# Shinokawa/Fast-SCNN-pytorch

Hardware: AMD Instinct MI355X
Metric: images/sec fwd+bwd @1024x2048 bs=8 per GPU; 1/2/4/8-GPU scaling (higher is better)
Workload: dtype bf16; 1 GPU; cfg3 train step: fwd + CE(ignore -1) + bwd + fused SGD (fused low-res upsample+CE head); model=FastSCNN (19 classes), global_batch=8, per_gpu_batch=8, parallelism=dp1

## Files before the change

### fast-scnn-pytorch_amd/_lib.py

```python
import ctypes
import os
import threading

_HERE = os.path.dirname(os.path.abspath(__file__))
LIB_PATH = os.environ.get("FSCNN_LIB", os.path.join(_HERE, "libfastscnn_hip.so"))

DT_F32, DT_BF16, DT_F16 = 0, 1, 2
DT_U8 = 3

c_int, c_ll, c_float, c_vp, c_char_p = (ctypes.c_int, ctypes.c_longlong, ctypes.c_float,
                                        ctypes.c_void_p, ctypes.c_char_p)
c_ull, c_double = ctypes.c_ulonglong, ctypes.c_double
P_int, P_ll, P_vp = ctypes.POINTER(c_int), ctypes.POINTER(c_ll), ctypes.POINTER(c_vp)
P_float = ctypes.POINTER(c_float)
P_double = ctypes.POINTER(c_double)
c_uint, P_ubyte = ctypes.c_uint, ctypes.POINTER(ctypes.c_ubyte)


class AuxHead(ctypes.Structure):
    _fields_ = [("head", c_int), ("aux_weight", c_float), ("ignore_index", c_ll),
                ("smooth", c_float), ("dice_weight", c_float), ("focal_weight", c_float),
                ("alpha", c_float), ("gamma", c_float), ("thresh", c_float), ("min_kept", c_ll),
                ("class_weight", c_vp)]

# ... 146 lines not shown
                                       c_vp]),
    "fscnn_block_ir_fwd": (c_int, [c_vp, c_int, c_int, c_int, c_int, c_int, c_int, c_int, c_int,
                                   c_vp, c_vp, c_vp, c_vp, c_vp, c_vp, c_vp, c_vp, c_vp, c_int,
                                   c_vp, c_int, c_vp]),
    "fscnn_pyramid_pool_bwd": (c_int, [c_vp, c_int, c_int, c_int, c_int, c_int, c_vp, c_int,
                                       c_int, c_vp]),
    "fscnn_bn_apply": (c_int, [c_ll, c_int, c_vp, c_int, c_vp, c_vp, c_vp, c_int, c_vp, c_vp, c_vp,
                               c_int, c_int, c_vp, c_int, c_int, c_vp]),
    "fscnn_bn_bwd": (c_int, [c_ll, c_int, c_vp, c_int, c_vp, c_int, c_vp, c_vp, c_vp, c_vp, c_vp,
                             c_int, c_int, c_vp, c_vp, c_vp, c_vp, c_vp, c_vp, c_vp, c_vp, c_vp,
                             c_vp, c_vp, c_vp, c_vp, c_int, P_int, P_int, c_vp]),
    "fscnn_ppm_branches_ok": (c_int, [c_int, c_int, c_int]),
    "fscnn_ppm_branches_fwd": (c_int, [c_int, P_int, c_int, c_vp, c_vp, c_vp, c_vp, c_vp, c_vp,
                                       c_vp, c_float, c_vp, c_vp, c_int, c_vp, c_vp, c_vp, c_vp,
                                       c_int, c_vp]),
    "fscnn_ppm_branches_bwd": (c_int, [c_int, P_int, c_int, c_vp, c_int, c_vp, c_int, c_vp, c_vp,
                                       c_vp, c_vp, c_vp, c_vp, c_vp, c_vp, c_vp, c_vp, c_vp, c_int,
                                       c_vp]),
    "fscnn_ppm_up_fwd": (c_int, [c_vp, c_int, c_int, c_int, c_int, c_vp, c_int, c_int, c_vp]),
    "fscnn_ppm_up_bwd": (c_int, [c_vp, c_int, c_int, c_int, c_int, c_int, c_int, c_vp, c_vp]),
    "fscnn_dropout": (c_int, [c_vp, c_int, c_int, c_int, c_int, c_int, c_int, c_ull, c_vp, c_ull,
                              c_float, c_vp, c_vp, c_vp, c_int, c_vp]),
    "fscnn_dw3x3_parts": (c_int, [c_int, c_int, c_int, c_int, c_int, c_int, c_int]),
    "fscnn_dw3x3_fwd_train": (c_int, [c_vp, c_int, c_int, c_int, c_int, c_int, c_int, c_vp, c_vp,
                                      c_vp, c_vp, c_vp, c_vp, c_vp, c_vp, c_vp, c_vp, c_vp, c_vp,
                                      c_float, c_vp, c_vp, c_vp, c_vp, P_int, c_vp]),
    "fscnn_dw3x3_dgrad_bn": (c_int, [c_vp, c_int, c_int, c_int, c_int, c_int, c_int, c_vp, c_vp,
                                     c_vp, c_vp, c_vp, c_vp, c_vp, c_int, c_vp, c_vp, c_vp, c_vp,
                                     c_vp, c_vp, P_int, c_vp]),
    "fscnn_dw3x3_wgrad_train": (c_int, [c_vp, c_vp, c_int, c_int, c_int, c_int, c_int, c_int,
                                        c_vp, c_vp, c_vp, c_vp, c_vp]),
    "fscnn_pw_fwd_train_route": (c_int, [c_int, c_int, c_int, c_int, c_int, c_int, c_int, P_int]),
    "fscnn_pw_fwd_train": (c_int, [c_int, c_int, c_int, c_vp, c_int, c_vp, c_vp, c_vp, c_int, c_vp,
                                   c_vp, c_int, c_vp, c_vp, c_vp, c_vp, c_vp, c_vp, c_vp, c_vp,
                                   c_float, c_vp, c_vp, c_vp, c_vp, c_int, P_int, P_int, c_vp]),
    "fscnn_pw_wgrad_train": (c_int, [c_int, c_int, c_int, c_vp, c_int, c_vp, c_int, c_vp, c_vp,
                                     c_vp, c_vp, c_vp, c_vp, c_int, P_int, c_vp]),
    "fscnn_pw_dgrad_train_route": (c_int, [c_int, c_int, c_int, c_int, c_int, c_int, c_int, c_int,
                                           P_int]),
    "fscnn_pw_dgrad_train": (c_int, [c_int, c_int, c_int, c_vp, c_int, c_vp, c_int, c_vp, c_int,
                                     c_vp, c_int, c_vp, c_int, c_vp, c_vp, c_vp, c_vp, c_int,
                                     c_vp, c_vp, c_vp, c_vp, c_vp, c_vp, c_vp, c_int, c_float,
                                     c_ull, c_ull, c_vp, c_int, P_int, P_int, c_vp]),
    "fscnn_im2col3": (c_int, [c_vp, c_int, c_int, c_int, c_int, c_int, c_int, c_vp, c_int, c_vp]),
    "fscnn_col2im3": (c_int, [c_vp, c_int, c_int, c_int, c_int, c_int, c_int, c_vp, c_int, c_int,
                              c_vp]),
# ... 74 lines not shown
```

### fast-scnn-pytorch_amd/csrc/capi.cpp

```cpp
#include <algorithm>
#include <chrono>
#include <cmath>
#include <cstdlib>
#include <cstdarg>
#include <cstdio>
#include <cstring>
#include <new>
#include <string>

#include "../../include/fastscnn.h"
#include "net.hpp"

namespace fscnn {

static thread_local char g_err[512] = "";

void set_error(const char* fmt, ...) {
  va_list ap;
  va_start(ap, fmt);
  vsnprintf(g_err, sizeof g_err, fmt, ap);
  va_end(ap);
}
const char* last_error() { return g_err; }

// ... 1541 lines not shown
  d.y = y; d.ldy = ldy; d.seed = seed; d.p = p; d.seed_add = seed_add;
  d.seed_ptr = reinterpret_cast<const uint64_t*>(seed_slot);
  return dropout(d, dtype, S(stream));
}

static int dw_train_check(const char* who, int dtype, int N, int H, int W, int C, int stride) {
  if (!dt_ok(dtype)) {
    set_error("%s: dtype %d", who, dtype);
    return E_INVALID;
  }
  const int V = vec_w(dtype);
  if (N < 1 || H < 1 || W < 1 || C < 1 || C % V || (stride != 1 && stride != 2)) {
    set_error("%s: N=%d H=%d W=%d C=%d stride=%d (C a multiple of %d, stride 1 or 2)", who, N, H,
              W, C, stride, V);
    return E_INVALID;
  }
  return OK;
}

int fscnn_dw3x3_parts(int N, int H, int W, int C, int stride, int dtype, int dgrad) {
  if (dw_train_check("fscnn_dw3x3_parts", dtype, N, H, W, C, stride)) return -1;
  if (dgrad) return dw_dgrad_parts(N, H, W, C, dtype, stride);
  return dw_parts(N, (H - 1) / stride + 1, (W - 1) / stride + 1, C, dtype, stride);
}

int fscnn_dw3x3_fwd_train(const void* x, int dtype, int N, int H, int W, int C, int stride,
                          const float* w, const float* in_scale, const float* in_shift, void* z,
                          float* part, unsigned* counters, double* tsum, const float* gamma,
                          const float* beta, float* rmean, float* rvar, long long* nbt,
                          float momentum, float* mean, float* invstd, float* scale, float* shift,
                          int* in_kernel, void* stream) {
  if (!x || !w || !z || !part || !counters || !tsum || !gamma || !beta || !rmean || !rvar ||
      !mean || !invstd || !scale || !shift || ((in_scale != nullptr) != (in_shift != nullptr))) {
    set_error("fscnn_dw3x3_fwd_train: null argument (in_scale and in_shift come together)");
    return E_INVALID;
  }
  const int rc = dw_train_check("fscnn_dw3x3_fwd_train", dtype, N, H, W, C, stride);
  if (rc) return rc;
  DwArgs d{};
  d.N = N; d.H = H; d.W = W; d.C = C; d.stride = stride;
  d.Ho = (H - 1) / stride + 1; d.Wo = (W - 1) / stride + 1;
  d.x = x; d.w = w; d.in_scale = in_scale; d.in_shift = in_shift;
  d.relu = 0; d.y = z;
  d.part = part;
  d.tail.counters = counters;
  d.tail.tsum = tsum;
// ... 526 lines not shown
```

### fast-scnn-pytorch_amd/csrc/dwconv.hip

```cpp
#include "bn_finish.hpp"

#include <optional>

namespace fscnn {

constexpr int DWL_CB = 8;

template <typename T, int S> struct DwCfg;
template <> struct DwCfg<float, 1> { static constexpr int HS = 2, WS = 4, GX = 8, GY = 4; };
template <> struct DwCfg<float, 2> { static constexpr int HS = 1, WS = 2, GX = 8, GY = 4; };
template <> struct DwCfg<bf16, 1> { static constexpr int HS = 2, WS = 4, GX = 4, GY = 4; };
template <> struct DwCfg<bf16, 2> { static constexpr int HS = 2, WS = 2, GX = 4, GY = 4; };
template <int S> struct DwCfg<f16, S> : DwCfg<bf16, S> {};
template <typename T, int S> struct DwTile {
  static constexpr int HS = DwCfg<T, S>::HS, WS = DwCfg<T, S>::WS;
  static constexpr int GX = DwCfg<T, S>::GX, GY = DwCfg<T, S>::GY, G = GX * GY;
  static constexpr int QPV = VecW<T>::V / 4;
  static constexpr int TH = GY * HS, TW = GX * WS;
  static constexpr int IR = (TH - 1) * S + 3, IC = (TW - 1) * S + 3;
  static constexpr int LPT = (IR * IC + QPV * G - 1) / (QPV * G);
  static constexpr int NR = (HS - 1) * S + 3, NC = (WS - 1) * S + 3;
};

__device__ __forceinline__ void quad_ld(const float* p, float (&v)[4]) {
// ... 56 lines not shown
    const int r = pix / G::IC, col = pix - r * G::IC;
    const int hi = hi0 + r, wi = wi0 + col;
    const bool ok = pix < G::IR * G::IC && hi >= 0 && hi < H && wi >= 0 && wi < W;
    const size_t off = ok ? (((size_t)n * H + hi) * W + wi) * C + (size_t)(cvbase + lv) * V : 0;
    raw[k] = sel4(ok, *reinterpret_cast<const uint4*>(x + off));
  }
#pragma unroll
  for (int k = 0; k < G::LPT; ++k) {
    const int i = tid + k * nthr;
    if (i < G::IR * G::IC * cbv) {
      uint4 v = raw[k];
      if constexpr (IT) {
        const int pix = i / cbv;
        const int r = pix / G::IC, col = pix - r * G::IC;
        const int hi = hi0 + r, wi = wi0 + col;
        const bool ok = hi >= 0 && hi < H && wi >= 0 && wi < W;
        v = sel4(ok, bnrelu_vec<T>(v, sc, sh));
      }
      s_in[i] = v;
    }
  }
}

template <typename T, int S, bool FLIP, bool IT, bool BR = false, bool TL = false>
__global__ __launch_bounds__(256, 3) void dw_fwd_kernel(DwArgs a, int cbv) {
  using G = DwTile<T, S>;
  extern __shared__ __attribute__((aligned(16))) uint4 s_dyn[];
  uint4* s_in = s_dyn;
  float* s_red = reinterpret_cast<float*>(s_dyn + G::IR * G::IC * cbv);
  const int tid = threadIdx.x, nthr = blockDim.x;
  const int QB = cbv * G::QPV;
  const int q = tid % QB, grp = tid / QB;
  const int gx = grp % G::GX, gy = grp / G::GX;
  int bx, by, bz;
  dw_tile(bx, by, bz);
  const int tiles_h = cdiv(a.Ho, G::TH);
  const int n = bz / tiles_h;
  const int th0 = (bz - n * tiles_h) * G::TH, tw0 = by * G::TW;
  const int c0 = bx * cbv * VecW<T>::V + q * 4;
  stamp(a.stamps, 0);
  dw_stage<T, S, IT>(s_in, (const T*)a.x, a.H, a.W, a.C, n, th0 * S - 1, tw0 * S - 1,
                     bx * cbv, cbv, tid, nthr, a.in_scale, a.in_shift);
  float wt[9][4];
#pragma unroll
  for (int j = 0; j < 4; ++j)
#pragma unroll
    for (int t = 0; t < 9; ++t) wt[FLIP ? 8 - t : t][j] = a.w[(size_t)(c0 + j) * 9 + t];
  __syncthreads();
  stamp(a.stamps, 1);

  const T* sl = reinterpret_cast<const T*>(s_in);
  const int pstride = cbv * VecW<T>::V;
  float acc[G::HS][G::WS][4];
#pragma unroll
  for (int r = 0; r < G::HS; ++r)
#pragma unroll
    for (int p = 0; p < G::WS; ++p)
#pragma unroll
      for (int j = 0; j < 4; ++j) acc[r][p][j] = 0.f;
  const int lr0 = gy * G::HS * S, lc0 = gx * G::WS * S;
#pragma unroll
  for (int rr = 0; rr < G::NR; ++rr) {
    asm volatile("" ::: "memory");
#pragma unroll
    for (int ci = 0; ci < G::NC; ++ci) {
      float v[4];
      quad_ld(sl + ((lr0 + rr) * G::IC + lc0 + ci) * pstride + q * 4, v);
#pragma unroll
      for (int r = 0; r < G::HS; ++r) {
        const int kh = rr - r * S;
        if (kh < 0 || kh > 2) continue;
#pragma unroll
        for (int p = 0; p < G::WS; ++p) {
          const int kw = ci - p * S;
          if (kw < 0 || kw > 2) continue;
#pragma unroll
          for (int j = 0; j < 4; ++j) acc[r][p][j] = fmaf(v[j], wt[kh * 3 + kw][j], acc[r][p][j]);
        }
      }
    }
  }

  const int ho0 = th0 + gy * G::HS, wo0 = tw0 + gx * G::WS;
  const int nrow = max(0, min(G::HS, a.Ho - ho0)), ncol = max(0, min(G::WS, a.Wo - wo0));
  {
    float sc[4], sh[4];
#pragma unroll
    for (int j = 0; j < 4; ++j) {
      sc[j] = a.scale ? a.scale[c0 + j] : 1.f;
      sh[j] = a.scale ? a.shift[c0 + j] : 0.f;
    }
#pragma unroll
    for (int r = 0; r < G::HS; ++r) {
      if (r >= nrow) continue;
      T* yb = (T*)a.y + (((size_t)n * a.Ho + ho0 + r) * a.Wo + wo0) * a.C + c0;
#pragma unroll
      for (int p = 0; p < G::WS; ++p) {
        if (p >= ncol) continue;
        float o[4];
#pragma unroll
        for (int j = 0; j < 4; ++j) {
          const float t = acc[r][p][j] * sc[j] + sh[j];
          o[j] = a.relu ? fmaxf(t, 0.f) : t;
          acc[r][p][j] = round_as<T>(o[j]);
        }
        quad_st(yb + (size_t)p * a.C, o);
      }
    }
  }
  stamp(a.stamps, 2);
  if constexpr (BR) {
    const BnBwdPart& b = a.bs;
    const bool m2 = b.mode == 2;
    float bm[4], bi[4], bsc[4], bsh[4], s1[4], s2[4];
#pragma unroll
    for (int j = 0; j < 4; ++j) {
      bm[j] = b.mean[c0 + j];
      bi[j] = b.invstd[c0 + j];
      bsc[j] = m2 ? b.scale[c0 + j] : 0.f;
      bsh[j] = m2 ? b.shift[c0 + j] : 1.f;
      s1[j] = s2[j] = 0.f;
    }
#pragma unroll
    for (int r = 0; r < G::HS; ++r) {
      float z[G::WS][4];
#pragma unroll
      for (int p = 0; p < G::WS; ++p) {
        const bool ok = r < nrow && p < ncol;
        const size_t pix = ok ? ((size_t)n * a.Ho + ho0 + r) * a.Wo + wo0 + p : 0;
        quad_ld((const T*)b.z + pix * a.C + c0, z[p]);
      }
#pragma unroll
      for (int p = 0; p < G::WS; ++p) {
        const bool ok = r < nrow && p < ncol;
#pragma unroll
        for (int j = 0; j < 4; ++j) {
          float gv = round_as<T>(acc[r][p][j]);
          gv = (ok && fmaf(z[p][j], bsc[j], bsh[j]) > 0.f) ? gv : 0.f;
          s1[j] += gv;
          s2[j] += gv * (z[p][j] - bm[j]) * bi[j];
        }
      }
      asm volatile("" ::: "memory");
    }
    float* rec = b.part + ((size_t)bz * gridDim.y + by) * 2 * a.C;
#pragma unroll
    for (int pass = 0; pass < 2; ++pass) {
      __syncthreads();
#pragma unroll
      for (int j = 0; j < 4; ++j) s_red[(grp * QB + q) * 4 + j] = pass ? s2[j] : s1[j];
      __syncthreads();
      if (grp == 0) {
#pragma unroll
        for (int j = 0; j < 4; ++j) {
          float t = 0.f;
          for (int g2 = 0; g2 < G::G; ++g2) t += s_red[(g2 * QB + q) * 4 + j];
          st_wt(rec + (size_t)pass * a.C + c0 + j, t);
        }
      }
    }
    stamp(a.stamps, 3);
    if constexpr (TL)
      tail_finish<false>(b.part, gridDim.y * gridDim.z, a.C, bz * gridDim.y + by,
                         bx * cbv * VecW<T>::V, cbv * VecW<T>::V, bx, a.tail,
                         reinterpret_cast<double*>(s_dyn));
    stamp(a.stamps, 4);
    return;
  }
  if (a.part == nullptr) return;
  const int trows = min(G::TH, a.Ho - th0), tcols = min(G::TW, a.Wo - tw0);
  const float cnt = (float)(trows * tcols);
  float mean[4];
#pragma unroll
  for (int j = 0; j < 4; ++j) {
    float sum = 0.f;
#pragma unroll
    for (int r = 0; r < G::HS; ++r)
#pragma unroll
      for (int p = 0; p < G::WS; ++p) sum += (r < nrow && p < ncol) ? acc[r][p][j] : 0.f;
    s_red[(grp * QB + q) * 4 + j] = sum;
  }
  __syncthreads();
#pragma unroll
  for (int j = 0; j < 4; ++j) {
    float sum = 0.f;
    for (int g = 0; g < G::G; ++g) sum += s_red[(g * QB + q) * 4 + j];
    mean[j] = sum / cnt;
  }
  __syncthreads();
#pragma unroll
  for (int j = 0; j < 4; ++j) {
    float m2 = 0.f;
#pragma unroll
    for (int r = 0; r < G::HS; ++r)
#pragma unroll
      for (int p = 0; p < G::WS; ++p) {
        const float d = acc[r][p][j] - mean[j];
        m2 += (r < nrow && p < ncol) ? d * d : 0.f;
      }
    s_red[(grp * QB + q) * 4 + j] = m2;
  }
  __syncthreads();
  if (grp == 0) {
    float* rec = a.part + ((size_t)bz * gridDim.y + by) * 3 * a.C;
#pragma unroll
    for (int j = 0; j < 4; ++j) {
      float m2 = 0.f;
      for (int g = 0; g < G::G; ++g) m2 += s_red[(g * QB + q) * 4 + j];
      st_wt(rec + c0 + j, mean[j]);
      st_wt(rec + a.C + c0 + j, m2);
      st_wt(rec + 2 * a.C + c0 + j, cnt);
    }
  }
  stamp(a.stamps, 3);
  if constexpr (TL)
    tail_finish<true>(a.part, gridDim.y * gridDim.z, a.C, bz * gridDim.y + by,
                      bx * cbv * VecW<T>::V, cbv * VecW<T>::V, bx, a.tail,
                      reinterpret_cast<double*>(s_dyn));
  stamp(a.stamps, 4);
}

template <typename T, int S>
static size_t dw_shm(int cbv) {
  using G = DwTile<T, S>;
  return (size_t)G::IR * G::IC * cbv * 16 + (size_t)cbv * 32 * 16;
}

static dim3 dw_grid(int N, int Ho, int Wo, int C, int V, int S, int& cbv) {
  cbv = dw_cbv(C / V);
  int TH, TW;
  if (V == 4) {
    TH = S == 1 ? DwTile<float, 1>::TH : DwTile<float, 2>::TH;
    TW = S == 1 ? DwTile<float, 1>::TW : DwTile<float, 2>::TW;
  } else {
    TH = S == 1 ? DwTile<bf16, 1>::TH : DwTile<bf16, 2>::TH;
    TW = S == 1 ? DwTile<bf16, 1>::TW : DwTile<bf16, 2>::TW;
  }
  return dim3(C / V / cbv, cdiv(Wo, TW), N * cdiv(Ho, TH));
}

int dw_parts(int N, int Ho, int Wo, int C, int dtype, int stride) {
  int cbv;
  dim3 g = dw_grid(N, Ho, Wo, C, dtype == DT_F32 ? 4 : 8, stride, cbv);
  return (int)(g.y * g.z);
}

template <typename T, bool FLIP, bool IT, bool BR>
static void dw_launch_fwd_t(const DwArgs& a, dim3 grid, int nthr, int cbv, hipStream_t st) {
  if constexpr (BR) {
    if (a.tail_ink) prof_launch(dw_fwd_kernel<T, 1, true, false, true, true>, grid, nthr, dw_shm<T, 1>(cbv), st, a, cbv);
    else prof_launch(dw_fwd_kernel<T, 1, true, false, true>, grid, nthr, dw_shm<T, 1>(cbv), st, a, cbv);
    return;
  }
  if (!FLIP && a.tail_ink) {
    if (a.stride == 1) prof_launch(dw_fwd_kernel<T, 1, false, IT, false, true>, grid, nthr, dw_shm<T, 1>(cbv), st, a, cbv);
    else prof_launch(dw_fwd_kernel<T, 2, false, IT, false, true>, grid, nthr, dw_shm<T, 2>(cbv), st, a, cbv);
    return;
  }
  if (a.stride == 1) prof_launch(dw_fwd_kernel<T, 1, FLIP, IT>, grid, nthr, dw_shm<T, 1>(cbv), st, a, cbv);
  else prof_launch(dw_fwd_kernel<T, 2, FLIP, IT>, grid, nthr, dw_shm<T, 2>(cbv), st, a, cbv);
}

template <bool FLIP, bool IT, bool BR = false>
static int dw_launch_fwd(const DwArgs& a, int dtype, hipStream_t st) {
  const int V = dtype == DT_F32 ? 4 : 8;
  int cbv;
  dim3 grid = dw_grid(a.N, a.Ho, a.Wo, a.C, V, a.stride, cbv);
  if (grid.z > 65535 || grid.y > 65535) {
    set_error("dw: grid too large (%u x %u)", grid.y, grid.z);
    return E_UNSUPPORTED;
  }
  const int nthr = cbv * 32;
  DwArgs as = a;
  as.stamps = stamp_region();
  if (dtype == DT_F32) dw_launch_fwd_t<float, FLIP, IT, BR>(as, grid, nthr, cbv, st);
  else if (dtype == DT_F16) dw_launch_fwd_t<f16, FLIP, IT, BR>(as, grid, nthr, cbv, st);
  else dw_launch_fwd_t<bf16, FLIP, IT, BR>(as, grid, nthr, cbv, st);
  return check_launch(FLIP ? "dw_dgrad" : "dw_fwd");
}

int dw_fwd_tail_ink(const DwArgs& a, int dtype, int* P) {
  int cbv;
  const dim3 g = dw_grid(a.N, a.Ho, a.Wo, a.C, dtype == DT_F32 ? 4 : 8, a.stride, cbv);
// ... 248 lines not shown
    else DWD2(bf16);
#undef DWD2
    rc = check_launch("dw_dgrad");
  }
  if (rc || !fin || ink) return rc;
  ps.reset();
  return bn_bwd_finalize(a.bs.part, P, a.C, a.tail.count, a.tail.dgamma, a.tail.dbeta,
                         a.tail.coef, st, a.tail.counters, a.tail.tab);
}

int dw_dgrad_parts(int N, int H, int W, int C, int dtype, int stride) {
  const int V = dtype == DT_F32 ? 4 : 8;
  if (stride == 1) {
    int cbv;
    const dim3 g = dw_grid(N, H, W, C, V, 1, cbv);
    return (int)(g.y * g.z);
  }
  int bx, by;
  dw_block_shape(C, DWD2_V, bx, by);
  const int gy = cdiv(W, by * 4), NB = N * ((H + 1) / 2);
  return gy * cdiv(NB, dwd2_rpw(gy, NB));
}

template <typename T, int S, bool IT>
__global__ __launch_bounds__(256, 2) void dw_wgrad_kernel(DwBwdArgs a, int cbv, int tpb) {
  using G = DwTile<T, S>;
  extern __shared__ __attribute__((aligned(16))) uint4 s_in[];
  const int tid = threadIdx.x, nthr = blockDim.x;
  const int QB = cbv * G::QPV;
  const int q = tid % QB, grp = tid / QB;
  const int gx = grp % G::GX, gy = grp / G::GX;
  int bx, by, bz;
  dw_tile(bx, by, bz);
  const int tiles_h = cdiv(a.Ho, G::TH), tiles_w = cdiv(a.Wo, G::TW);
  const int n = bz / tiles_h;
  const int th0 = (bz - n * tiles_h) * G::TH;
  const int c0 = bx * cbv * VecW<T>::V + q * 4;
  const int ho0 = th0 + gy * G::HS;
  const int nrow = max(0, min(G::HS, a.Ho - ho0));
  const T* sl = reinterpret_cast<const T*>(s_in);
  const int pstride = cbv * VecW<T>::V;
  float acc[9][4];
#pragma unroll
  for (int t = 0; t < 9; ++t)
#pragma unroll
    for (int j = 0; j < 4; ++j) acc[t][j] = 0.f;
  const int tw_lo = by * tpb, tw_hi = min(tiles_w, tw_lo + tpb);
  for (int twi = tw_lo; twi < tw_hi; ++twi) {
    const int tw0 = twi * G::TW;
    const int wo0 = tw0 + gx * G::WS;
    const int ncol = max(0, min(G::WS, a.Wo - wo0));
    float g[G::HS][G::WS][4];
    const T* gb = (const T*)a.dy + c0;
#pragma unroll
    for (int r = 0; r < G::HS; ++r)
#pragma unroll
      for (int p = 0; p < G::WS; ++p) {
        const bool ok = r < nrow && p < ncol;
        const size_t off = ok ? (((size_t)n * a.Ho + ho0 + r) * a.Wo + wo0 + p) * a.C : 0;
        quad_ld(gb + off, g[r][p]);
      }
#pragma unroll
    for (int r = 0; r < G::HS; ++r)
#pragma unroll
      for (int p = 0; p < G::WS; ++p) {
        const bool ok = r < nrow && p < ncol;
#pragma unroll
        for (int j = 0; j < 4; ++j) g[r][p][j] = ok ? g[r][p][j] : 0.f;
      }
    __syncthreads();
    dw_stage<T, S, IT>(s_in, (const T*)a.x, a.H, a.W, a.C, n, th0 * S - 1, tw0 * S - 1, bx * cbv,
                       cbv, tid, nthr, a.x_scale, a.x_shift);
    __syncthreads();
    const int lr0 = gy * G::HS * S, lc0 = gx * G::WS * S;
#pragma unroll
    for (int rr = 0; rr < G::NR; ++rr)
#pragma unroll
      for (int ci = 0; ci < G::NC; ++ci) {
        float v[4];
        quad_ld(sl + ((lr0 + rr) * G::IC + lc0 + ci) * pstride + q * 4, v);
#pragma unroll
        for (int r = 0; r < G::HS; ++r) {
          const int kh = rr - r * S;
          if (kh < 0 || kh > 2) continue;
#pragma unroll
          for (int p = 0; p < G::WS; ++p) {
            const int kw = ci - p * S;
            if (kw < 0 || kw > 2) continue;
#pragma unroll
            for (int j = 0; j < 4; ++j)
              acc[kh * 3 + kw][j] = fmaf(v[j], g[r][p][j], acc[kh * 3 + kw][j]);
          }
        }
      }
  }
// ... 23 lines not shown
  long long tpb = blocks / 1024;
  if (tpb < 1) tpb = 1;
  if (tpb > tiles_w) tpb = tiles_w;
  grid.y = (unsigned)cdiv((int)tiles_w, (int)tpb);
  return (int)tpb;
}

int dw_wgrad_parts(int N, int Ho, int Wo, int C, int dtype, int stride) {
  dim3 g;
  int cbv;
  dw_wgrad_tpb(N, Ho, Wo, C, dtype == DT_F32 ? 4 : 8, stride, g, cbv);
  return (int)(g.y * g.z);
}

int dw_wgrad(const DwBwdArgs& a, int dtype, hipStream_t st) {
  const int V = dtype == DT_F32 ? 4 : 8;
  dim3 grid;
  int cbv;
  const int tpb = dw_wgrad_tpb(a.N, a.Ho, a.Wo, a.C, V, a.stride, grid, cbv);
  const double E = dtype == DT_F32 ? 4.0 : 2.0;
  const double in_el = (double)a.N * a.C * a.H * a.W, out_el = (double)a.N * a.C * a.Ho * a.Wo;
  ProfScope ps(PK_DW_WGRAD, st, E * (in_el + out_el), 18.0 * out_el);
  const int nthr = cbv * 32;
#define DWW_LAUNCH(T, S)                                                                      \
  do {                                                                                        \
    if (a.x_scale) prof_launch(dw_wgrad_kernel<T, S, true>, grid, nthr, dw_shm<T, S>(cbv), st, a, cbv, tpb); \
    else prof_launch(dw_wgrad_kernel<T, S, false>, grid, nthr, dw_shm<T, S>(cbv), st, a, cbv, tpb);          \
  } while (0)
  if (dtype == DT_F32) {
    if (a.stride == 1) DWW_LAUNCH(float, 1);
    else DWW_LAUNCH(float, 2);
  } else if (dtype == DT_F16) {
    if (a.stride == 1) DWW_LAUNCH(f16, 1);
    else DWW_LAUNCH(f16, 2);
  } else {
    if (a.stride == 1) DWW_LAUNCH(bf16, 1);
    else DWW_LAUNCH(bf16, 2);
  }
#undef DWW_LAUNCH
  return check_launch("dw_wgrad");
}

int dw_wgrad_reduce(float* slab, int P, int C, float* dw, hipStream_t st) {
  return reduce_slabs_ex(slab, P, 9LL * C, 9LL * C, dw, 0, C, st);
}

}
```

### fast-scnn-pytorch_amd/csrc/kernels.hpp

```cpp
#pragma once
#include "common.hpp"

namespace fscnn {

constexpr int MAX_FOLD = 48;
constexpr double BN_FROZEN_COUNT = -1.0;


struct Conv0Args {
  const void* x;
  int x_bf16;
  int N, H, W, Ho, Wo;
  const float* w;
  const float* scale;
  const float* shift;
  int relu;
  void* y;
  float* part;
  unsigned long long* stamps = nullptr;
};

struct Conv0WgradArgs {
  const void* x;
  int x_bf16;
// ... 475 lines not shown
int conv0_fwd(const Conv0Args& a, int y_dtype, hipStream_t st);
int conv0_wgrad_parts(int N, int Ho, int Wo, int rows_per_block);
int conv0_wgrad(const Conv0WgradArgs& a, int dz_dtype, hipStream_t st);

constexpr int LC0_SLAB = 2 * 864 + 27;
struct LtdC0BwdArgs {
  int N, H, W;
  int Ho, Wo;
  const void* dy;
  const float* w;
  BnBwdPart bs{};
  BnTail tail{};
  const void* x;
  int x_dtype, XH, XW;
  float* slab;
};
int ltd_c0_bwd_parts(int N, int H, int W);
bool ltd_c0_bwd_ok(int dtype, int x_dtype, int XW, const void* x);
int ltd_c0_bwd(const LtdC0BwdArgs& a, int dtype, hipStream_t st);
int conv0_wgrad_combine(const float* sums, const float* tab, const float* mean, float* dw,
                        hipStream_t st);

int dw_parts(int N, int Ho, int Wo, int C, int dtype, int stride);
int dw_fwd(const DwArgs& a, int dtype, hipStream_t st);
int dw_dgrad(const DwBwdArgs& a, int dtype, hipStream_t st);
int dw_dgrad_parts(int N, int H, int W, int C, int dtype, int stride);
int dw_fwd_tail_ink(const DwArgs& a, int dtype, int* P);
int dw_dgrad_tail_ink(const DwBwdArgs& a, int dtype, int* P);
int dw_wgrad_parts(int N, int Ho, int Wo, int C, int dtype, int stride);
int dw_wgrad(const DwBwdArgs& a, int dtype, hipStream_t st);
int dw_wgrad_reduce(float* slab, int P, int C, float* dw, hipStream_t st);

int gemm_parts(int M);
int gemm_nt(const GemmArgs& a, int dtype, hipStream_t st);
bool gemm_stream_ok(const GemmArgs& a, int dtype);
int gemm_stream(const GemmArgs& a, int dtype, hipStream_t st);
int gemm_stream_parts(const GemmArgs& a, int dtype);
int gemm_nt_parts(const GemmArgs& a, int dtype);
int gemm_nt_tail_ink(const GemmArgs& a, int dtype, int* P);
int gemm_tn_splits(int M, int N, int K);
int gemm_tn(GemmTnArgs a, int splits, int dtype, hipStream_t st);
int reduce_slabs(float* slab, int S, long long stride, long long count, float* out,
                 int accumulate, hipStream_t st);
int reduce_slabs_ex(float* slab, int S, long long stride, long long count, float* out,
                    int accumulate, int C9, hipStream_t st);
constexpr int RED_MAXJOBS = 64;
// ... 167 lines not shown
```

### include/fastscnn.h

```cpp
#ifndef FASTSCNN_H
#define FASTSCNN_H

#ifdef __cplusplus
extern "C" {
#endif

typedef struct fscnn_net fscnn_net;
typedef struct fscnn_plan fscnn_plan;

const char* fscnn_version(void);
const char* fscnn_last_error(void);

int fscnn_net_create(int num_classes, int aux, fscnn_net** out);
void fscnn_net_destroy(fscnn_net* net);
int fscnn_net_param_count(const fscnn_net* net, int* count, long long* total_floats);
int fscnn_net_param_info(const fscnn_net* net, int i, const char** name, long long* offset,
                         long long* numel);
int fscnn_net_buffer_count(const fscnn_net* net, int* count, long long* total_floats, int* num_bn);
int fscnn_net_buffer_info(const fscnn_net* net, int i, const char** name, long long* offset,
                          long long* numel);
int fscnn_net_stage_range(const fscnn_net* net, int stage, long long* begin, long long* end);

int fscnn_plan_create(const fscnn_net* net, int N, int H, int W, int dtype, int train,
                      fscnn_plan** out);
// ... 313 lines not shown
                 const float* mean2, const float* invstd2, const float* scale2, float* part,
                 unsigned* counters, void* dz, void* dz2, float* dgamma, float* dbeta,
                 float* dgamma2, float* dbeta2, float* coef, int dtype, int* P,
                 int* rows_per_block, void* stream);
int fscnn_ppm_branches_ok(int maxM, int K, int dtype);
int fscnn_ppm_branches_fwd(int nb, const int* M, int K, const void* x, const void* w,
                           const float* gamma, const float* beta, float* rmean, float* rvar,
                           long long* nbt, float momentum, void* z, void* y, int ldy, float* mean,
                           float* invstd, float* scale, float* shift, int dtype, void* stream);
int fscnn_ppm_branches_bwd(int nb, const int* M, int K, const void* dy, int lddy, const void* y,
                           int ldy, const void* z, const float* mean, const float* invstd,
                           const float* scale, const float* gamma, const void* x, const void* w,
                           float* dgamma, float* dbeta, float* dw, void* dx, int dtype,
                           void* stream);
int fscnn_ppm_up_fwd(const void* feats, int dtype, int N, int H, int W, void* y, int ldy, int coff,
                     void* stream);
int fscnn_ppm_up_bwd(const void* dy, int dtype, int N, int H, int W, int ldy, int coff,
                     void* dfeats, void* stream);
int fscnn_dropout(const void* x, int ldx, int dtype, int N, int H, int W, int C,
                  unsigned long long seed, const unsigned long long* seed_slot,
                  unsigned long long seed_add, float p, const float* x_scale,
                  const float* x_shift, void* y, int ldy, void* stream);
int fscnn_dw3x3_parts(int N, int H, int W, int C, int stride, int dtype, int dgrad);
int fscnn_dw3x3_fwd_train(const void* x, int dtype, int N, int H, int W, int C, int stride,
                          const float* w, const float* in_scale, const float* in_shift, void* z,
                          float* part, unsigned* counters, double* tsum, const float* gamma,
                          const float* beta, float* rmean, float* rvar, long long* nbt,
                          float momentum, float* mean, float* invstd, float* scale, float* shift,
                          int* in_kernel, void* stream);
int fscnn_dw3x3_dgrad_bn(const void* dy, int dtype, int N, int H, int W, int C, int stride,
                         const float* w, void* dx, const void* z, const float* mean,
                         const float* invstd, const float* scale, const float* shift,
                         int relu_mode, float* part, unsigned* counters, double* tsum,
                         float* dgamma, float* dbeta, float* coef, int* in_kernel, void* stream);
int fscnn_dw3x3_wgrad_train(const void* x, const void* dy, int dtype, int N, int H, int W, int C,
                            int stride, const float* x_scale, const float* x_shift, float* slab,
                            float* dw, void* stream);

int fscnn_pw_fwd_train_route(int M, int N, int K, int lda, int ldc, int lazy, int dtype,
                             int* records);
int fscnn_pw_fwd_train(int M, int N, int K, const void* A, int lda, const float* a_scale,
                       const float* a_shift, const void* B, int ldb, const float* bias, void* z,
                       int ldc, float* part, unsigned* counters, double* tsum, const float* gamma,
                       const float* beta, float* rmean, float* rvar, long long* nbt,
                       float momentum, float* mean, float* invstd, float* scale, float* shift,
                       int dtype, int* route, int* records, void* stream);
// ... 23 lines not shown
```

Measured before the change: 1471 images/s.

## Specialise depthwise 3x3 fwd/wgrad kernels on compile-time channel width with interior fast path

Adds compile-time channel-block-width (CBV) variants of the depthwise 3x3 forward and weight-gradient kernels, used when the width is 4/6/8 and pointers are aligned. These variants stage input with precomputed 32-bit byte offsets, load weights and BN params as float4, and take a separate branch for interior tiles that skips bounds checks. They also remap block indices via dw_tile32. This targets address arithmetic, predication and scalar loads, at the cost of more template instantiations, possible register pressure, and 32-bit offset overflow limits guarded by a size check.

```diff
diff --git a/fast-scnn-pytorch_amd/_lib.py b/fast-scnn-pytorch_amd/_lib.py
--- a/fast-scnn-pytorch_amd/_lib.py
+++ b/fast-scnn-pytorch_amd/_lib.py
@@ -192,6 +192,7 @@
     "fscnn_dropout": (c_int, [c_vp, c_int, c_int, c_int, c_int, c_int, c_int, c_ull, c_vp, c_ull,
                               c_float, c_vp, c_vp, c_vp, c_int, c_vp]),
     "fscnn_dw3x3_parts": (c_int, [c_int, c_int, c_int, c_int, c_int, c_int, c_int]),
+    "fscnn_dw3x3_ct_width": (c_int, [c_int, c_int, c_int, c_int, c_int, c_int]),
     "fscnn_dw3x3_fwd_train": (c_int, [c_vp, c_int, c_int, c_int, c_int, c_int, c_int, c_vp, c_vp,
                                       c_vp, c_vp, c_vp, c_vp, c_vp, c_vp, c_vp, c_vp, c_vp, c_vp,
                                       c_float, c_vp, c_vp, c_vp, c_vp, P_int, c_vp]),
diff --git a/fast-scnn-pytorch_amd/csrc/capi.cpp b/fast-scnn-pytorch_amd/csrc/capi.cpp
--- a/fast-scnn-pytorch_amd/csrc/capi.cpp
+++ b/fast-scnn-pytorch_amd/csrc/capi.cpp
@@ -1587,6 +1587,11 @@
   if (dw_train_check("fscnn_dw3x3_parts", dtype, N, H, W, C, stride)) return -1;
   if (dgrad) return dw_dgrad_parts(N, H, W, C, dtype, stride);
   return dw_parts(N, (H - 1) / stride + 1, (W - 1) / stride + 1, C, dtype, stride);
+}
+
+int fscnn_dw3x3_ct_width(int N, int H, int W, int C, int stride, int dtype) {
+  if (dw_train_check("fscnn_dw3x3_ct_width", dtype, N, H, W, C, stride)) return -1;
+  return dw_ct_width(N, (H - 1) / stride + 1, (W - 1) / stride + 1, W, C, dtype, stride);
 }
 
 int fscnn_dw3x3_fwd_train(const void* x, int dtype, int N, int H, int W, int C, int stride,
diff --git a/fast-scnn-pytorch_amd/csrc/dwconv.hip b/fast-scnn-pytorch_amd/csrc/dwconv.hip
--- a/fast-scnn-pytorch_amd/csrc/dwconv.hip
+++ b/fast-scnn-pytorch_amd/csrc/dwconv.hip
@@ -1,5 +1,6 @@
 #include "bn_finish.hpp"
 
+#include <initializer_list>
 #include <optional>
 
 namespace fscnn {
@@ -102,30 +103,133 @@
   }
 }
 
-template <typename T, int S, bool FLIP, bool IT, bool BR = false, bool TL = false>
-__global__ __launch_bounds__(256, 3) void dw_fwd_kernel(DwArgs a, int cbv) {
+
+__device__ __forceinline__ void dw_tile32(int& cx, int& cy, int& cz) {
+  const unsigned gx = gridDim.x, gy = gridDim.y, gz = gridDim.z;
+  const unsigned T = gx * gy * gz;
+  unsigned L = blockIdx.x + gx * (blockIdx.y + gy * blockIdx.z);
+  if ((T & 7u) == 0) L = (L & 7u) * (T >> 3) + (L >> 3);
+  cx = (int)(L % gx);
+  const unsigned r = L / gx;
+  cy = (int)(r % gy);
+  cz = (int)(r / gy);
+}
+
+template <bool VEC>
+__device__ __forceinline__ void ch4(const float* p, int c, float (&v)[4]) {
+  if constexpr (VEC) {
+    const float4 t = *reinterpret_cast<const float4*>(p + c);
+    v[0] = t.x; v[1] = t.y; v[2] = t.z; v[3] = t.w;
+  } else {
+#pragma unroll
+    for (int j = 0; j < 4; ++j) v[j] = p[c + j];
+  }
+}
+
+__device__ __forceinline__ float mul_rn(float x, float y) {
+#pragma clang fp contract(off)
+  return x * y;
+}
+
+template <typename T, int S, bool IT, int CBV, bool INT>
+__device__ __forceinline__ void dw_stage_ct(uint4* s_in, const char* xb, uint32_t rowb,
+                                            uint32_t pixb, int H, int W, int hi0, int wi0,
+                                            int cvbase, int tid, const float* isc,
+                                            const float* ish) {
   using G = DwTile<T, S>;
-  extern __shared__ __attribute__((aligned(16))) uint4 s_dyn[];
+  constexpr int V = VecW<T>::V;
+  constexpr int NPIX = G::IR * G::IC, DR = 32 / G::IC, DC = 32 % G::IC;
+  const int lv = tid % CBV, pix0 = tid / CBV;
+  float sc[IT ? V : 1], sh[IT ? V : 1];
+  if constexpr (IT) {
+    const int cb = (cvbase + lv) * V;
+#pragma unroll
+    for (int j = 0; j < V; j += 4) {
+      const float4 s4 = *reinterpret_cast<const float4*>(isc + cb + j);
+      const float4 h4 = *reinterpret_cast<const float4*>(ish + cb + j);
+      sc[j] = s4.x; sc[j + 1] = s4.y; sc[j + 2] = s4.z; sc[j + 3] = s4.w;
+      sh[j] = h4.x; sh[j + 1] = h4.y; sh[j + 2] = h4.z; sh[j + 3] = h4.w;
+    }
+  }
+  const uint32_t safe = (INT ? 0u : rowb + pixb) + (uint32_t)lv * 16u;
+  uint4 raw[G::LPT];
+  bool okk[G::LPT];
+  int r = pix0 / G::IC, col = pix0 - r * G::IC;
+  uint32_t off = (uint32_t)r * rowb + (uint32_t)col * pixb + (uint32_t)lv * 16u;
+#pragma unroll
+  for (int k = 0; k < G::LPT; ++k) {
+    bool ok = (32 * k + 31 < NPIX) || pix0 + 32 * k < NPIX;
+    if constexpr (!INT)
+      ok = ok && (unsigned)(hi0 + r) < (unsigned)H && (unsigned)(wi0 + col) < (unsigned)W;
+    okk[k] = ok;
+    const uint4 t = *reinterpret_cast<const uint4*>(xb + (ok ? off : safe));
+    if constexpr (INT) raw[k] = t;
+    else raw[k] = sel4(ok, t);
+    const bool wrap = col + DC >= G::IC;
+    col += wrap ? DC - G::IC : DC;
+    r += wrap ? DR + 1 : DR;
+    off += wrap ? (uint32_t)(DR + 1) * rowb - (uint32_t)(G::IC - DC) * pixb
+                : (uint32_t)DR * rowb + (uint32_t)DC * pixb;
+  }
+#pragma unroll
+  for (int k = 0; k < G::LPT; ++k) {
+    if ((32 * k + 31 < NPIX) || pix0 + 32 * k < NPIX) {
+      uint4 v = raw[k];
+      if constexpr (IT) {
+        if constexpr (INT) v = bnrelu_vec<T>(v, sc, sh);
+        else v = sel4(okk[k], bnrelu_vec<T>(v, sc, sh));
+      }
+      s_in[tid + k * 32 * CBV] = v;
+    }
+  }
+}
+
+template <typename T, int S, bool FLIP, bool IT, bool BR, int CBV, bool INT>
+__device__ __forceinline__ void dw_fwd_body(const DwArgs& a, int cbv_rt, uint4* s_dyn, int bx,
+                                            int by, int bz, int n, int th0, int tw0) {
+  using G = DwTile<T, S>;
+  constexpr bool CT = CBV > 0;
+  const int cbv = CT ? CBV : cbv_rt;
   uint4* s_in = s_dyn;
   float* s_red = reinterpret_cast<float*>(s_dyn + G::IR * G::IC * cbv);
   const int tid = threadIdx.x, nthr = blockDim.x;
   const int QB = cbv * G::QPV;
   const int q = tid % QB, grp = tid / QB;
   const int gx = grp % G::GX, gy = grp / G::GX;
-  int bx, by, bz;
-  dw_tile(bx, by, bz);
-  const int tiles_h = cdiv(a.Ho, G::TH);
-  const int n = bz / tiles_h;
-  const int th0 = (bz - n * tiles_h) * G::TH, tw0 = by * G::TW;
   const int c0 = bx * cbv * VecW<T>::V + q * 4;
+  const uint32_t orowb = (uint32_t)a.Wo * (uint32_t)a.C * (uint32_t)sizeof(T);
+  const uint32_t opixb = (uint32_t)a.C * (uint32_t)sizeof(T);
+  const size_t obase = ((((size_t)n * a.Ho + th0) * a.Wo + tw0) * a.C + (size_t)bx * cbv * VecW<T>::V) * sizeof(T);
+  const uint32_t olane = (uint32_t)(gy * G::HS) * orowb + (uint32_t)(gx * G::WS) * opixb +
+                         (uint32_t)q * 4u * (uint32_t)sizeof(T);
   stamp(a.stamps, 0);
-  dw_stage<T, S, IT>(s_in, (const T*)a.x, a.H, a.W, a.C, n, th0 * S - 1, tw0 * S - 1,
-                     bx * cbv, cbv, tid, nthr, a.in_scale, a.in_shift);
   float wt[9][4];
-#pragma unroll
-  for (int j = 0; j < 4; ++j)
-#pragma unroll
-    for (int t = 0; t < 9; ++t) wt[FLIP ? 8 - t : t][j] = a.w[(size_t)(c0 + j) * 9 + t];
+  if constexpr (CT) {
+    const long long xoff = ((((long long)n * a.H + (th0 * S - 1)) * a.W + (tw0 * S - 1)) * a.C +
+                            (long long)bx * cbv * VecW<T>::V) * (long long)sizeof(T);
+    dw_stage_ct<T, S, IT, CBV, INT>(s_in, (const char*)a.x + xoff,
+                                    (uint32_t)a.W * (uint32_t)a.C * (uint32_t)sizeof(T),
+                                    (uint32_t)a.C * (uint32_t)sizeof(T), a.H, a.W, th0 * S - 1,
+                                    tw0 * S - 1, bx * cbv, tid, a.in_scale, a.in_shift);
+    const float4* wp = reinterpret_cast<const float4*>(a.w + (size_t)c0 * 9);
+#pragma unroll
+    for (int i = 0; i < 9; ++i) {
+      const float4 t4 = wp[i];
+      const float tt[4] = {t4.x, t4.y, t4.z, t4.w};
+#pragma unroll
+      for (int e = 0; e < 4; ++e) {
+        const int f = 4 * i + e;
+        wt[FLIP ? 8 - f % 9 : f % 9][f / 9] = tt[e];
+      }
+    }
+  } else {
+    dw_stage<T, S, IT>(s_in, (const T*)a.x, a.H, a.W, a.C, n, th0 * S - 1, tw0 * S - 1,
+                       bx * cbv, cbv, tid, nthr, a.in_scale, a.in_shift);
+#pragma unroll
+    for (int j = 0; j < 4; ++j)
+#pragma unroll
+      for (int t = 0; t < 9; ++t) wt[FLIP ? 8 - t : t][j] = a.w[(size_t)(c0 + j) * 9 + t];
+  }
   __syncthreads();
   stamp(a.stamps, 1);
 
@@ -159,24 +263,37 @@
         }
       }
     }
-  }
+    if constexpr (CT) {
+#pragma unroll
+      for (int r = 0; r < G::HS; ++r)
+#pragma unroll
+        for (int p = 0; p < G::WS; ++p) {
+          typedef float pair_t __attribute__((ext_vector_type(2)));
+          pair_t lo = {acc[r][p][0], acc[r][p][1]}, hi = {acc[r][p][2], acc[r][p][3]};
+          asm volatile("" : "+v"(lo), "+v"(hi));
+          acc[r][p][0] = lo.x; acc[r][p][1] = lo.y; acc[r][p][2] = hi.x; acc[r][p][3] = hi.y;
+        }
+    }
+  }
+  asm volatile("" ::: "memory");
 
   const int ho0 = th0 + gy * G::HS, wo0 = tw0 + gx * G::WS;
-  const int nrow = max(0, min(G::HS, a.Ho - ho0)), ncol = max(0, min(G::WS, a.Wo - wo0));
+  const int nrow = INT ? G::HS : max(0, min(G::HS, a.Ho - ho0));
+  const int ncol = INT ? G::WS : max(0, min(G::WS, a.Wo - wo0));
   {
-    float sc[4], sh[4];
-#pragma unroll
-    for (int j = 0; j < 4; ++j) {
-      sc[j] = a.scale ? a.scale[c0 + j] : 1.f;
-      sh[j] = a.scale ? a.shift[c0 + j] : 0.f;
-    }
+    float sc[4] = {1.f, 1.f, 1.f, 1.f}, sh[4] = {0.f, 0.f, 0.f, 0.f};
+    if (a.scale) {
+      ch4<CT>(a.scale, c0, sc);
+      ch4<CT>(a.shift, c0, sh);
+    }
+    char* const ytile = (char*)a.y + obase;
 #pragma unroll
     for (int r = 0; r < G::HS; ++r) {
-      if (r >= nrow) continue;
+      if (!INT && r >= nrow) continue;
       T* yb = (T*)a.y + (((size_t)n * a.Ho + ho0 + r) * a.Wo + wo0) * a.C + c0;
 #pragma unroll
       for (int p = 0; p < G::WS; ++p) {
-        if (p >= ncol) continue;
+        if (!INT && p >= ncol) continue;
         float o[4];
 #pragma unroll
         for (int j = 0; j < 4; ++j) {
@@ -184,7 +301,10 @@
           o[j] = a.relu ? fmaxf(t, 0.f) : t;
           acc[r][p][j] = round_as<T>(o[j]);
         }
-        quad_st(yb + (size_t)p * a.C, o);
+        if constexpr (CT)
+          quad_st(reinterpret_cast<T*>(ytile + (olane + (uint32_t)r * orowb + (uint32_t)p * opixb)), o);
+        else
+          quad_st(yb + (size_t)p * a.C, o);
       }
     }
   }
@@ -192,27 +312,33 @@
   if constexpr (BR) {
     const BnBwdPart& b = a.bs;
     const bool m2 = b.mode == 2;
-    float bm[4], bi[4], bsc[4], bsh[4], s1[4], s2[4];
-#pragma unroll
-    for (int j = 0; j < 4; ++j) {
-      bm[j] = b.mean[c0 + j];
-      bi[j] = b.invstd[c0 + j];
-      bsc[j] = m2 ? b.scale[c0 + j] : 0.f;
-      bsh[j] = m2 ? b.shift[c0 + j] : 1.f;
-      s1[j] = s2[j] = 0.f;
-    }
+    float bm[4], bi[4], bsc[4] = {0.f, 0.f, 0.f, 0.f}, bsh[4] = {1.f, 1.f, 1.f, 1.f}, s1[4], s2[4];
+    ch4<CT>(b.mean, c0, bm);
+    ch4<CT>(b.invstd, c0, bi);
+    if (m2) {
+      ch4<CT>(b.scale, c0, bsc);
+      ch4<CT>(b.shift, c0, bsh);
+    }
+#pragma unroll
+    for (int j = 0; j < 4; ++j) s1[j] = s2[j] = 0.f;
+    const char* const ztile = (const char*)b.z + obase;
 #pragma unroll
     for (int r = 0; r < G::HS; ++r) {
       float z[G::WS][4];
 #pragma unroll
       for (int p = 0; p < G::WS; ++p) {
-        const bool ok = r < nrow && p < ncol;
-        const size_t pix = ok ? ((size_t)n * a.Ho + ho0 + r) * a.Wo + wo0 + p : 0;
-        quad_ld((const T*)b.z + pix * a.C + c0, z[p]);
+        const bool ok = INT || (r < nrow && p < ncol);
+        if constexpr (CT) {
+          const uint32_t zo = (uint32_t)r * orowb + (uint32_t)p * opixb + olane;
+          quad_ld(reinterpret_cast<const T*>(ztile + (ok ? zo : (uint32_t)q * 4u * (uint32_t)sizeof(T))), z[p]);
+        } else {
+          const size_t pix = ok ? ((size_t)n * a.Ho + ho0 + r) * a.Wo + wo0 + p : 0;
+          quad_ld((const T*)b.z + pix * a.C + c0, z[p]);
+        }
       }
 #pragma unroll
       for (int p = 0; p < G::WS; ++p) {
-        const bool ok = r < nrow && p < ncol;
+        const bool ok = INT || (r < nrow && p < ncol);
 #pragma unroll
         for (int j = 0; j < 4; ++j) {
           float gv = round_as<T>(acc[r][p][j]);
@@ -240,11 +366,6 @@
       }
     }
     stamp(a.stamps, 3);
-    if constexpr (TL)
-      tail_finish<false>(b.part, gridDim.y * gridDim.z, a.C, bz * gridDim.y + by,
-                         bx * cbv * VecW<T>::V, cbv * VecW<T>::V, bx, a.tail,
-                         reinterpret_cast<double*>(s_dyn));
-    stamp(a.stamps, 4);
     return;
   }
   if (a.part == nullptr) return;
@@ -276,7 +397,7 @@
 #pragma unroll
       for (int p = 0; p < G::WS; ++p) {
         const float d = acc[r][p][j] - mean[j];
-        m2 += (r < nrow && p < ncol) ? d * d : 0.f;
+        m2 += (r < nrow && p < ncol) ? mul_rn(d, d) : 0.f;
       }
     s_red[(grp * QB + q) * 4 + j] = m2;
   }
@@ -293,10 +414,38 @@
     }
   }
   stamp(a.stamps, 3);
-  if constexpr (TL)
-    tail_finish<true>(a.part, gridDim.y * gridDim.z, a.C, bz * gridDim.y + by,
-                      bx * cbv * VecW<T>::V, cbv * VecW<T>::V, bx, a.tail,
-                      reinterpret_cast<double*>(s_dyn));
+}
+
+template <typename T, int S, bool FLIP, bool IT, bool BR = false, bool TL = false, int CBV = 0>
+__global__ __launch_bounds__(256, 3) void dw_fwd_kernel(DwArgs a, int cbv_rt) {
+  using G = DwTile<T, S>;
+  extern __shared__ __attribute__((aligned(16))) uint4 s_dyn[];
+  int bx, by, bz;
+  if constexpr (CBV > 0) dw_tile32(bx, by, bz);
+  else dw_tile(bx, by, bz);
+  const int tiles_h = cdiv(a.Ho, G::TH);
+  const int n = bz / tiles_h;
+  const int th0 = (bz - n * tiles_h) * G::TH, tw0 = by * G::TW;
+  if constexpr (CBV > 0) {
+    const bool inside = th0 >= 1 && tw0 >= 1 && th0 * S - 1 + G::IR <= a.H &&
+                        tw0 * S - 1 + G::IC <= a.W && th0 + G::TH <= a.Ho && tw0 + G::TW <= a.Wo;
+    if (inside) dw_fwd_body<T, S, FLIP, IT, BR, CBV, true>(a, cbv_rt, s_dyn, bx, by, bz, n, th0, tw0);
+    else dw_fwd_body<T, S, FLIP, IT, BR, CBV, false>(a, cbv_rt, s_dyn, bx, by, bz, n, th0, tw0);
+  } else {
+    dw_fwd_body<T, S, FLIP, IT, BR, 0, false>(a, cbv_rt, s_dyn, bx, by, bz, n, th0, tw0);
+  }
+  if (!BR && a.part == nullptr) return;
+  if constexpr (TL) {
+    const int cbv = CBV > 0 ? CBV : cbv_rt;
+    if constexpr (BR)
+      tail_finish<false>(a.bs.part, gridDim.y * gridDim.z, a.C, bz * gridDim.y + by,
+                         bx * cbv * VecW<T>::V, cbv * VecW<T>::V, bx, a.tail,
+                         reinterpret_cast<double*>(s_dyn));
+    else
+      tail_finish<true>(a.part, gridDim.y * gridDim.z, a.C, bz * gridDim.y + by,
+                        bx * cbv * VecW<T>::V, cbv * VecW<T>::V, bx, a.tail,
+                        reinterpret_cast<double*>(s_dyn));
+  }
   stamp(a.stamps, 4);
 }
 
@@ -325,20 +474,57 @@
   return (int)(g.y * g.z);
 }
 
+static bool dw_generic() {
+  static const bool on = env_on("FSCNN_DW_GENERIC", false);
+  return on;
+}
+
+static bool dw_al16(const void* p) { return (uintptr_t)p % 16 == 0; }
+
+static bool dw_ct_ok(int cbv, int V, dim3 grid, int W, int Wo, int C,
+                     std::initializer_list<const float*> rows) {
+  if (dw_generic()) return false;
+  if (!(cbv == 8 || cbv == 6 || (cbv == 4 && V == 8))) return false;
+  if ((unsigned long long)grid.x * grid.y * grid.z >= (1ull << 31)) return false;
+  if (20LL * ((W > Wo ? W : Wo) + 80LL) * C * 4 >= (1LL << 31)) return false;
+  for (const float* r : rows)
+    if (!dw_al16(r)) return false;
+  return true;
+}
+
+int dw_ct_width(int N, int Ho, int Wo, int W, int C, int dtype, int stride) {
+  const int V = dtype == DT_F32 ? 4 : 8;
+  int cbv;
+  const dim3 g = dw_grid(N, Ho, Wo, C, V, stride, cbv);
+  return dw_ct_ok(cbv, V, g, W, Wo, C, {}) ? cbv : 0;
+}
+
+template <typename T, bool FLIP, bool IT, bool BR, int CBV>
+static void dw_launch_fwd_c(const DwArgs& a, dim3 grid, int nthr, int cbv, hipStream_t st) {
+  if constexpr (BR) {
+    if (a.tail_ink) prof_launch(dw_fwd_kernel<T, 1, true, false, true, true, CBV>, grid, nthr, dw_shm<T, 1>(cbv), st, a, cbv);
+    else prof_launch(dw_fwd_kernel<T, 1, true, false, true, false, CBV>, grid, nthr, dw_shm<T, 1>(cbv), st, a, cbv);
+    return;
+  }
+  if (!FLIP && a.tail_ink) {
+    if (a.stride == 1) prof_launch(dw_fwd_kernel<T, 1, false, IT, false, true, CBV>, grid, nthr, dw_shm<T, 1>(cbv), st, a, cbv);
+    else prof_launch(dw_fwd_kernel<T, 2, false, IT, false, true, CBV>, grid, nthr, dw_shm<T, 2>(cbv), st, a, cbv);
+    return;
+  }
+  if (a.stride == 1) prof_launch(dw_fwd_kernel<T, 1, FLIP, IT, false, false, CBV>, grid, nthr, dw_shm<T, 1>(cbv), st, a, cbv);
+  else prof_launch(dw_fwd_kernel<T, 2, FLIP, IT, false, false, CBV>, grid, nthr, dw_shm<T, 2>(cbv), st, a, cbv);
+}
+
 template <typename T, bool FLIP, bool IT, bool BR>
 static void dw_launch_fwd_t(const DwArgs& a, dim3 grid, int nthr, int cbv, hipStream_t st) {
-  if constexpr (BR) {
-    if (a.tail_ink) prof_launch(dw_fwd_kernel<T, 1, true, false, true, true>, grid, nthr, dw_shm<T, 1>(cbv), st, a, cbv);
-    else prof_launch(dw_fwd_kernel<T, 1, true, false, true>, grid, nthr, dw_shm<T, 1>(cbv), st, a, cbv);
-    return;
-  }
-  if (!FLIP && a.tail_ink) {
-    if (a.stride == 1) prof_launch(dw_fwd_kernel<T, 1, false, IT, false, true>, grid, nthr, dw_shm<T, 1>(cbv), st, a, cbv);
-    else prof_launch(dw_fwd_kernel<T, 2, false, IT, false, true>, grid, nthr, dw_shm<T, 2>(cbv), st, a, cbv);
-    return;
-  }
-  if (a.stride == 1) prof_launch(dw_fwd_kernel<T, 1, FLIP, IT>, grid, nthr, dw_shm<T, 1>(cbv), st, a, cbv);
-  else prof_launch(dw_fwd_kernel<T, 2, FLIP, IT>, grid, nthr, dw_shm<T, 2>(cbv), st, a, cbv);
+  const bool ct = dw_ct_ok(cbv, VecW<T>::V, grid, a.W, a.Wo, a.C,
+                           {a.w, a.in_scale, a.in_shift, a.scale, a.shift, a.bs.mean, a.bs.invstd,
+                            a.bs.scale, a.bs.shift});
+  if (ct && cbv == 8) return dw_launch_fwd_c<T, FLIP, IT, BR, 8>(a, grid, nthr, cbv, st);
+  if (ct && cbv == 6) return dw_launch_fwd_c<T, FLIP, IT, BR, 6>(a, grid, nthr, cbv, st);
+  if constexpr (sizeof(T) == 2)
+    if (ct && cbv == 4) return dw_launch_fwd_c<T, FLIP, IT, BR, 4>(a, grid, nthr, cbv, st);
+  dw_launch_fwd_c<T, FLIP, IT, BR, 0>(a, grid, nthr, cbv, st);
 }
 
 template <bool FLIP, bool IT, bool BR = false>
@@ -633,16 +819,72 @@
   return gy * cdiv(NB, dwd2_rpw(gy, NB));
 }
 
-template <typename T, int S, bool IT>
-__global__ __launch_bounds__(256, 2) void dw_wgrad_kernel(DwBwdArgs a, int cbv, int tpb) {
+template <typename T, int S, bool IT, int CBV, bool INT>
+__device__ __forceinline__ void dw_wgrad_load(const DwBwdArgs& a, int cbv, uint4* s_in,
+                                              float (&g)[DwTile<T, S>::HS][DwTile<T, S>::WS][4],
+                                              int bx, int n, int th0, int tw0, int q, int gx, int gy,
+                                              int c0, int nrow_b) {
+  using G = DwTile<T, S>;
+  constexpr bool CT = CBV > 0;
+  const int tid = threadIdx.x, nthr = blockDim.x;
+  const int ho0 = th0 + gy * G::HS, wo0 = tw0 + gx * G::WS;
+  const int nrow = INT ? G::HS : nrow_b;
+  const int ncol = INT ? G::WS : max(0, min(G::WS, a.Wo - wo0));
+  const uint32_t orowb = (uint32_t)a.Wo * (uint32_t)a.C * (uint32_t)sizeof(T);
+  const uint32_t opixb = (uint32_t)a.C * (uint32_t)sizeof(T);
+  const size_t obase = ((((size_t)n * a.Ho + th0) * a.Wo + tw0) * a.C + (size_t)bx * cbv * VecW<T>::V) * sizeof(T);
+  const uint32_t qb = (uint32_t)q * 4u * (uint32_t)sizeof(T);
+  const uint32_t olane = (uint32_t)(gy * G::HS) * orowb + (uint32_t)(gx * G::WS) * opixb + qb;
+  const T* gb = (const T*)a.dy + c0;
+#pragma unroll
+  for (int r = 0; r < G::HS; ++r)
+#pragma unroll
+    for (int p = 0; p < G::WS; ++p) {
+      const bool ok = INT || (r < nrow && p < ncol);
+      if constexpr (CT) {
+        const uint32_t go = (uint32_t)r * orowb + (uint32_t)p * opixb + olane;
+        quad_ld(reinterpret_cast<const T*>((const char*)a.dy + obase + (size_t)(ok ? go : qb)), g[r][p]);
+      } else {
+        const size_t off = ok ? (((size_t)n * a.Ho + ho0 + r) * a.Wo + wo0 + p) * a.C : 0;
+        quad_ld(gb + off, g[r][p]);
+      }
+    }
+  if constexpr (!INT) {
+#pragma unroll
+    for (int r = 0; r < G::HS; ++r)
+#pragma unroll
+      for (int p = 0; p < G::WS; ++p) {
+        const bool ok = r < nrow && p < ncol;
+#pragma unroll
+        for (int j = 0; j < 4; ++j) g[r][p][j] = ok ? g[r][p][j] : 0.f;
+      }
+  }
+  __syncthreads();
+  if constexpr (CT) {
+    const long long xoff = ((((long long)n * a.H + (th0 * S - 1)) * a.W + (tw0 * S - 1)) * a.C +
+                            (long long)bx * cbv * VecW<T>::V) * (long long)sizeof(T);
+    dw_stage_ct<T, S, IT, CBV, INT>(s_in, (const char*)a.x + xoff,
+                                    (uint32_t)a.W * (uint32_t)a.C * (uint32_t)sizeof(T),
+                                    (uint32_t)a.C * (uint32_t)sizeof(T), a.H, a.W, th0 * S - 1,
+                                    tw0 * S - 1, bx * cbv, tid, a.x_scale, a.x_shift);
+  } else {
+    dw_stage<T, S, IT>(s_in, (const T*)a.x, a.H, a.W, a.C, n, th0 * S - 1, tw0 * S - 1, bx * cbv,
+                       cbv, tid, nthr, a.x_scale, a.x_shift);
+  }
+}
+
+template <typename T, int S, bool IT, int CBV = 0>
+__global__ __launch_bounds__(256, 2) void dw_wgrad_kernel(DwBwdArgs a, int cbv_rt, int tpb) {
   using G = DwTile<T, S>;
   extern __shared__ __attribute__((aligned(16))) uint4 s_in[];
-  const int tid = threadIdx.x, nthr = blockDim.x;
+  const int cbv = CBV > 0 ? CBV : cbv_rt;
+  const int tid = threadIdx.x;
   const int QB = cbv * G::QPV;
   const int q = tid % QB, grp = tid / QB;
   const int gx = grp % G::GX, gy = grp / G::GX;
   int bx, by, bz;
-  dw_tile(bx, by, bz);
+  if constexpr (CBV > 0) dw_tile32(bx, by, bz);
+  else dw_tile(bx, by, bz);
   const int tiles_h = cdiv(a.Ho, G::TH), tiles_w = cdiv(a.Wo, G::TW);
   const int n = bz / tiles_h;
   const int th0 = (bz - n * tiles_h) * G::TH;
@@ -657,31 +899,17 @@
 #pragma unroll
     for (int j = 0; j < 4; ++j) acc[t][j] = 0.f;
   const int tw_lo = by * tpb, tw_hi = min(tiles_w, tw_lo + tpb);
+  const bool rows_in = th0 >= 1 && th0 * S - 1 + G::IR <= a.H && th0 + G::TH <= a.Ho;
   for (int twi = tw_lo; twi < tw_hi; ++twi) {
     const int tw0 = twi * G::TW;
-    const int wo0 = tw0 + gx * G::WS;
-    const int ncol = max(0, min(G::WS, a.Wo - wo0));
     float g[G::HS][G::WS][4];
-    const T* gb = (const T*)a.dy + c0;
-#pragma unroll
-    for (int r = 0; r < G::HS; ++r)
-#pragma unroll
-      for (int p = 0; p < G::WS; ++p) {
-        const bool ok = r < nrow && p < ncol;
-        const size_t off = ok ? (((size_t)n * a.Ho + ho0 + r) * a.Wo + wo0 + p) * a.C : 0;
-        quad_ld(gb + off, g[r][p]);
-      }
-#pragma unroll
-    for (int r = 0; r < G::HS; ++r)
-#pragma unroll
-      for (int p = 0; p < G::WS; ++p) {
-        const bool ok = r < nrow && p < ncol;
-#pragma unroll
-        for (int j = 0; j < 4; ++j) g[r][p][j] = ok ? g[r][p][j] : 0.f;
-      }
-    __syncthreads();
-    dw_stage<T, S, IT>(s_in, (const T*)a.x, a.H, a.W, a.C, n, th0 * S - 1, tw0 * S - 1, bx * cbv,
-                       cbv, tid, nthr, a.x_scale, a.x_shift);
+    if constexpr (CBV > 0) {
+      const bool inside = rows_in && tw0 >= 1 && tw0 * S - 1 + G::IC <= a.W && tw0 + G::TW <= a.Wo;
+      if (inside) dw_wgrad_load<T, S, IT, CBV, true>(a, cbv, s_in, g, bx, n, th0, tw0, q, gx, gy, c0, nrow);
+      else dw_wgrad_load<T, S, IT, CBV, false>(a, cbv, s_in, g, bx, n, th0, tw0, q, gx, gy, c0, nrow);
+    } else {
+      dw_wgrad_load<T, S, IT, 0, false>(a, cbv, s_in, g, bx, n, th0, tw0, q, gx, gy, c0, nrow);
+    }
     __syncthreads();
     const int lr0 = gy * G::HS * S, lc0 = gx * G::WS * S;
 #pragma unroll
@@ -751,10 +979,18 @@
   const double in_el = (double)a.N * a.C * a.H * a.W, out_el = (double)a.N * a.C * a.Ho * a.Wo;
   ProfScope ps(PK_DW_WGRAD, st, E * (in_el + out_el), 18.0 * out_el);
   const int nthr = cbv * 32;
+  const bool ct = dw_ct_ok(cbv, V, grid, a.W, a.Wo, a.C, {a.x_scale, a.x_shift});
+#define DWW_LAUNCH_C(T, S, CB)                                                                \
+  do {                                                                                        \
+    if (a.x_scale) prof_launch(dw_wgrad_kernel<T, S, true, CB>, grid, nthr, dw_shm<T, S>(cbv), st, a, cbv, tpb); \
+    else prof_launch(dw_wgrad_kernel<T, S, false, CB>, grid, nthr, dw_shm<T, S>(cbv), st, a, cbv, tpb);          \
+  } while (0)
 #define DWW_LAUNCH(T, S)                                                                      \
   do {                                                                                        \
-    if (a.x_scale) prof_launch(dw_wgrad_kernel<T, S, true>, grid, nthr, dw_shm<T, S>(cbv), st, a, cbv, tpb); \
-    else prof_launch(dw_wgrad_kernel<T, S, false>, grid, nthr, dw_shm<T, S>(cbv), st, a, cbv, tpb);          \
+    if (ct && cbv == 8) DWW_LAUNCH_C(T, S, 8);                                                \
+    else if (ct && cbv == 6) DWW_LAUNCH_C(T, S, 6);                                           \
+    else if (ct && cbv == 4 && sizeof(T) == 2) DWW_LAUNCH_C(T, S, (sizeof(T) == 2 ? 4 : 0));  \
+    else DWW_LAUNCH_C(T, S, 0);                                                               \
   } while (0)
   if (dtype == DT_F32) {
     if (a.stride == 1) DWW_LAUNCH(float, 1);
@@ -767,6 +1003,7 @@
     else DWW_LAUNCH(bf16, 2);
   }
 #undef DWW_LAUNCH
+#undef DWW_LAUNCH_C
   return check_launch("dw_wgrad");
 }
 
diff --git a/fast-scnn-pytorch_amd/csrc/kernels.hpp b/fast-scnn-pytorch_amd/csrc/kernels.hpp
--- a/fast-scnn-pytorch_amd/csrc/kernels.hpp
+++ b/fast-scnn-pytorch_amd/csrc/kernels.hpp
@@ -521,6 +521,7 @@
                         hipStream_t st);
 
 int dw_parts(int N, int Ho, int Wo, int C, int dtype, int stride);
+int dw_ct_width(int N, int Ho, int Wo, int W, int C, int dtype, int stride);
 int dw_fwd(const DwArgs& a, int dtype, hipStream_t st);
 int dw_dgrad(const DwBwdArgs& a, int dtype, hipStream_t st);
 int dw_dgrad_parts(int N, int H, int W, int C, int dtype, int stride);
diff --git a/include/fastscnn.h b/include/fastscnn.h
--- a/include/fastscnn.h
+++ b/include/fastscnn.h
@@ -359,6 +359,7 @@
                   unsigned long long seed_add, float p, const float* x_scale,
                   const float* x_shift, void* y, int ldy, void* stream);
 int fscnn_dw3x3_parts(int N, int H, int W, int C, int stride, int dtype, int dgrad);
+int fscnn_dw3x3_ct_width(int N, int H, int W, int C, int stride, int dtype);
 int fscnn_dw3x3_fwd_train(const void* x, int dtype, int N, int H, int W, int C, int stride,
                           const float* w, const float* in_scale, const float* in_shift, void* z,
                           float* part, unsigned* counters, double* tsum, const float* gamma,
```

Measured after the change: 1506 images/s (median of 6 runs). 2.4% higher.
